# kasirershahartau/tissue_image_processing

Hardware: AMD Instinct MI355X
Metric: frames/sec end-to-end (2048^2, z=30) (higher is better)
Workload: dtype f32(f16x3)

## Files before the change

### tissue_image_processing_amd/csrc/tip_core.hip

```cpp
#include "tip_internal.h"
#include <algorithm>
#include <cmath>
#include <cstdlib>
#include <map>
#include <mutex>

namespace tip {

static thread_local Ctx *g_ctx = nullptr;
static thread_local int g_requested_device = 0;

static int ctx_create(int device)
{
    Ctx *c = new Ctx();
    c->device = device;
    hipError_t e = hipSetDevice(device);
    if (e != hipSuccess) {
        c->err = std::string("hipSetDevice failed: ") + hipGetErrorString(e);
        g_ctx = c;
        return TIP_ERR_HIP;
    }
    {
        const char *pr = getenv("TIP_STREAM_PRIORITY");
        int lo = 0, hi = 0;
// ... 107 lines not shown
namespace {
Tuning g_tuning;
std::once_flag g_tuning_once;
std::mutex g_tuning_mu;

bool tuning_assign(Tuning &t, const char *name, const char *value)
{
    const Tuning def;
    const bool unset = !value || !*value;
    auto flag = [&](int &field, int dflt) { field = unset ? dflt : (strcmp(value, "0") != 0 ? 1 : 0); };
    auto num = [&](int &field, int dflt) { field = unset ? dflt : atoi(value); };
    auto pair = [&](int &a, int &b, int da, int db) {
        a = da; b = db;
        if (!unset) sscanf(value, "%d,%d", &a, &b);
    };
    const std::string n(name ? name : "");
    if (n == "TIP_WS_TIES") {
        if (unset) t.ws_ties = def.ws_ties;
        else t.ws_ties = (!strcmp(value, "fast") || !strcmp(value, "0")) ? 0 : 1;
    }
    else if (n == "TIP_WS_OPEN") pair(t.ws_open_a, t.ws_open_b, def.ws_open_a, def.ws_open_b);
    else if (n == "TIP_WS_NO_SKIP") flag(t.ws_no_skip, 0);
    else if (n == "TIP_WS_DEBUG") flag(t.ws_debug, 0);
    else if (n == "TIP_WS_NO_ENDGAME") flag(t.ws_no_endgame, 0);
    else if (n == "TIP_WS_NO_WIDE") flag(t.ws_no_wide, 0);
    else if (n == "TIP_PROJECT_GENERIC") flag(t.project_generic, 0);
    else if (n == "TIP_PROJECT_UNFUSED_PREBLUR") flag(t.project_unfused_preblur, 0);
    else if (n == "TIP_PROJECT_UNFUSED_MASK") flag(t.project_unfused_mask, 0);
    else if (n == "TIP_PROJECT_EXACT_SCORE") flag(t.project_exact_score, 0);
    else if (n == "TIP_PROJECT_DEBUG") flag(t.project_debug, 0);
    else if (n == "TIP_UNET_TILE8") num(t.unet_tile8, def.unet_tile8);
    else if (n == "TIP_UF_ONE_LEVEL") flag(t.uf_one_level, 0);
    else if (n == "TIP_UNET_SPB") num(t.unet_spb, def.unet_spb);
    else if (n == "TIP_UNET_XCD_MAP") flag(t.unet_xcd_map, 1);
    else if (n == "TIP_UNET_TAIL_UNFUSED") flag(t.unet_tail_unfused, 0);
    else if (n == "TIP_MB_SMALL") num(t.mb_small, def.mb_small);
    else if (n == "TIP_MB_BATCH") num(t.mb_batch, def.mb_batch);
    else return false;
    return true;
}

const char *const TUNING_NAMES[] = {"TIP_WS_TIES", "TIP_WS_OPEN", "TIP_WS_NO_SKIP", "TIP_WS_DEBUG", "TIP_WS_NO_ENDGAME", "TIP_WS_NO_WIDE",
                                    "TIP_PROJECT_GENERIC", "TIP_PROJECT_UNFUSED_PREBLUR", "TIP_PROJECT_UNFUSED_MASK",
                                    "TIP_PROJECT_EXACT_SCORE", "TIP_PROJECT_DEBUG", "TIP_UNET_TILE8", "TIP_UNET_TAIL_UNFUSED", "TIP_UNET_XCD_MAP", "TIP_UNET_SPB", "TIP_UF_ONE_LEVEL", "TIP_MB_SMALL", "TIP_MB_BATCH"};

void tuning_from_env()
{
    for (const char *name : TUNING_NAMES)
        if (const char *e = getenv(name)) tuning_assign(g_tuning, name, e);
}
}

const Tuning &tuning()
{
    std::call_once(g_tuning_once, tuning_from_env);
    return g_tuning;
}

int make_taps(Taps &t, const double *w, int n)
{
    if (n <= 0 || n > 255 || !(n & 1)) return fail(TIP_ERR_ARG, "tap count %d must be odd and <= 255", n);
    for (int i = 1; i <= n / 2; i++)
        if (fabs(w[n / 2 + i] - w[n / 2 - i]) > 2.220446049250313e-16)
            return fail(TIP_ERR_UNSUPPORTED, "only symmetric kernels (scipy's symmetric correlate1d branch)");
    memset(&t, 0, sizeof t);
    for (int i = 0; i < n; i++) t.w[i] = w[i];
    t.n = n;
    return TIP_OK;
}

static double np_pairwise_sum(const double *a, long n)
{
    if (n < 8) {
        double r = 0.0;
        for (long i = 0; i < n; i++) r += a[i];
        return r;
    } else if (n <= 128) {
// ... 207 lines not shown
```

### tissue_image_processing_amd/csrc/tip_internal.h

```cpp
#pragma once
#include <hip/hip_runtime.h>
#include <cstdarg>
#include <cstdint>
#include <cstdio>
#include <cstring>
#include <string>
#include <vector>
#include "../../include/tissue_hip.h"

namespace tip {

struct ProfRec { const char *name; hipEvent_t e0, e1; };

struct Ctx {
    int device = -1;
    hipStream_t stream = nullptr;
    std::string err;
    struct Block { void *p; size_t bytes; bool used; };
    std::vector<Block> pool;
    int last_ws_labels = 0;
    long last_ws_other = 0;
    hipEvent_t edge_event = nullptr;
    void *prep_ws = nullptr;
    void *pin_buf = nullptr;
// ... 6 lines not shown
Ctx &ctx();
int fail(int code, const char *fmt, ...);
void *ws_alloc(size_t bytes);
void *pinned_scratch(size_t bytes);
void ws_free(void *p);

struct WsGuard {
    std::vector<void *> ptrs;
    template <typename T> T *get(size_t count) {
        void *p = ws_alloc(count * sizeof(T) ? count * sizeof(T) : 16);
        if (p) ptrs.push_back(p);
        return (T *)p;
    }
    ~WsGuard() { for (void *p : ptrs) ws_free(p); }
};

void prof_begin(const char *name);
void prof_end();

struct Tuning {
    int ws_ties = 1;
    int ws_open_a = -1, ws_open_b = -1;
    int ws_no_skip = 0;
    int ws_debug = 0;
    int ws_no_endgame = 0, ws_no_wide = 0;
    int project_generic = 0, project_unfused_preblur = 0, project_unfused_mask = 0;
    int project_exact_score = 0, project_debug = 0;
    int unet_tail_unfused = 0;
    int unet_xcd_map = 1;
    int unet_spb = 3;
    int uf_one_level = 0;
    int mb_small = -1;
    int mb_batch = -1;
    int unet_tile8 = -1;
};
const Tuning &tuning();

#define TIP_HIP(call)                                                                             \
    do {                                                                                          \
        hipError_t e__ = (call);                                                                  \
        if (e__ != hipSuccess)                                                                    \
            return tip::fail(TIP_ERR_HIP, "%s failed: %s (%s:%d)", #call, hipGetErrorString(e__), \
                             __FILE__, __LINE__);                                                 \
    } while (0)

#define TIP_LAUNCH(name, kernel, grid, block, shmem, ...)                                  \
    do {                                                                                   \
        tip::prof_begin(name);                                                             \
        hipLaunchKernelGGL(kernel, grid, block, shmem, tip::ctx().stream, __VA_ARGS__);    \
        tip::prof_end();                                                                   \
        hipError_t e__ = hipGetLastError();                                                \
        if (e__ != hipSuccess)                                                             \
            return tip::fail(TIP_ERR_HIP, "launch %s: %s", name, hipGetErrorString(e__));  \
    } while (0)

static inline int cdiv(long a, long b) { return (int)((a + b - 1) / b); }

struct Taps {
    double w[256];
    int n;
};
struct TapsF {
    float w[256];
    int n;
};

// ... 9 lines not shown
```

### tissue_image_processing_amd/csrc/tip_unet.hip

```cpp
#include "tip_internal.h"
#include "tip_unet_conv.h"
#include <algorithm>
#include <atomic>

namespace tip {

__global__ void __launch_bounds__(256) k_bias_relu_affine_f32(float *__restrict__ x, const float *__restrict__ bias,
                                                              const float *__restrict__ scale, const float *__restrict__ shift,
                                                              long n4, int C)
{
    const long i = (long)blockIdx.x * blockDim.x + threadIdx.x;
    if (i >= n4) return;
    float4 v = reinterpret_cast<float4 *>(x)[i];
    const int c = (int)((i * 4) % C);
    const float4 b = *reinterpret_cast<const float4 *>(bias + c);
    const float4 s = *reinterpret_cast<const float4 *>(scale + c);
    const float4 t = *reinterpret_cast<const float4 *>(shift + c);
    v.x += b.x; v.y += b.y; v.z += b.z; v.w += b.w;
    v.x = v.x > 0.f ? v.x : 0.f; v.y = v.y > 0.f ? v.y : 0.f; v.z = v.z > 0.f ? v.z : 0.f; v.w = v.w > 0.f ? v.w : 0.f;
    v.x = v.x * s.x + t.x; v.y = v.y * s.y + t.y; v.z = v.z * s.z + t.z; v.w = v.w * s.w + t.w;
    reinterpret_cast<float4 *>(x)[i] = v;
}

int rankfilter2d_dev(const void *in, void *out, int dtype, int Y, int X, int ky, int kx, int fp, int border, int is_max);
// ... 380 lines not shown
    p.in0 = (const uint16_t *)d->in0; p.in1 = (const uint16_t *)(d->c1 > 0 ? d->in1 : d->in0);
    p.c0 = d->c0; p.c1 = d->c1; p.H = d->h; p.W = d->w;
    p.w = (const uint16_t *)d->weights; p.ntaps = d->ntaps;
    for (int t = 0; t < 9; ++t) {
        p.dy[t] = t < d->ntaps ? d->dy[t] : 0; p.dx[t] = t < d->ntaps ? d->dx[t] : 0;
        if (p.dy[t] < -1 || p.dy[t] > 1 || p.dx[t] < -1 || p.dx[t] > 1) return fail(TIP_ERR_ARG, "tip_unet_conv_dev: tap offsets are -1, 0 or 1");
    }
    p.cout = d->cout; p.bias = d->bias; p.scale = d->scale; p.shift = d->shift;
    p.out = (uint16_t *)d->out; p.outH = d->out_h; p.outW = d->out_w; p.sy = d->sy; p.sx = d->sx; p.oy = d->oy; p.ox = d->ox;
    p.pool_out = (uint16_t *)d->pool_out;
    p.acc_scale = d->format == 1 ? d->acc_scale : 1.f;
    for (int t = 0; t < 9; ++t) p.nmask[t] = d->tf ? (d->nmask[t] & 15) : 15;
    if (d->tf && (d->planes != 2 || d->ntaps != 4 || d->sy != 2 || d->sx != 2 || d->oy != 0 || d->ox != 0 || d->scale || d->pool_out || d->head_out ||
                  d->out_h != 2 * d->h || d->out_w != 2 * d->w))
        return fail(TIP_ERR_ARG, "tip_unet_conv_dev: the fused transposed convolution takes four offset taps, two planes, bias only, a 2h x 2w output");
#ifdef UC_TRACE
    static unsigned long long *trace_dev = nullptr;
    if (!trace_dev) { TIP_HIP(hipMalloc(&trace_dev, 1024)); }
    TIP_HIP(hipMemsetAsync(trace_dev, 0, 1024, (hipStream_t)stream));
    p.trace = trace_dev;
#endif
    p.head_w = d->head_w; p.head_b = d->head_b; p.head_out = d->head_out;
    if (d->head_out && (!d->head_w || !d->head_b || d->cout != UC_BN || !d->scale || d->pool_out || d->sy != 1 || d->sx != 1 || d->oy != 0 || d->ox != 0 ||
                        d->out_h != d->h || d->out_w != d->w))
        return fail(TIP_ERR_ARG, "tip_unet_conv_dev: the fused head needs a 128-channel Conv2D + BatchNorm layer with the plain output mapping");
    if (d->pool_out && (d->sy != 1 || d->sx != 1 || d->oy != 0 || d->ox != 0 || d->out_h != d->h || d->out_w != d->w))
        return fail(TIP_ERR_ARG, "tip_unet_conv_dev: pool_out needs the plain output mapping");
    const bool tf = d->tf != 0;
    const int t8 = tuning().unet_tile8;
    const bool want8 = t8 == 1 || (t8 < 0 && d->ntaps == 9 && d->c0 + d->c1 <= 128);
    const int th = (d->planes == 2 && d->h % 16 == 0 && !want8) ? 16 : 8;
    const int dist = (th == 16 && d->ntaps >= 4) ? 4 : 2;
    const int da = (th == 16 && d->ntaps <= 2) ? 2 : 1;
    const int threads = th * 32, hp = UC_HW * (th + 2);
    const int ntiles = (d->h / th) * (d->w / UC_TW), nblks = d->cout / UC_BN;
    p.xcd_map = (tuning().unet_xcd_map && nblks > 1 && ntiles % 8 == 0) ? 1 : 0;
    const dim3 grid = p.xcd_map ? dim3((unsigned)(ntiles * nblks)) : dim3(ntiles, nblks);
    const int a_per = (d->planes * ((hp * 2 + 63) / 64) * 64 + threads - 1) / threads;
    const int spb_want = tuning().unet_spb;
    const bool multi = th == 16 && dist == 4 && d->ntaps == 9 && spb_want > 1;
    const int spb = !multi ? 1 : (spb_want >= 3 ? 3 : ((((d->c0 + d->c1) / UC_KC) & 1) == 0 ? 2 : 1));
    const size_t lds = (size_t)(da + 1) * a_per * threads * 16 + (size_t)(spb > 1 ? 3 * spb : dist + 1) * d->planes * 256 * 16;
    hipStream_t s = (hipStream_t)stream;
    const int which = tf ? (th == 16 ? 7 : 8)
                         : d->planes == 3 ? 3 : (th == 16 ? (dist == 4 ? (spb == 3 ? 6 : (spb == 2 ? 5 : 2)) : (da == 2 ? 4 : 1)) : 0);
    static std::atomic<unsigned> attr_done[64];
    const unsigned bit = 1u << (which + (d->format ? 9 : 0));
    const int dev = c.device >= 0 && c.device < 64 ? c.device : 0;
#define UC_FLAVOUR(W, ...)                                                                                                                  \
    case W: {                                                                                                                               \
        if (!(attr_done[dev].load(std::memory_order_acquire) & bit)) {                                                                      \
            TIP_HIP(hipFuncSetAttribute((const void *)(__VA_ARGS__), hipFuncAttributeMaxDynamicSharedMemorySize, (int)lds));                \
            attr_done[dev].fetch_or(bit, std::memory_order_release);                                                                        \
        }                                                                                                                                   \
        hipLaunchKernelGGL((__VA_ARGS__), grid, dim3(threads), lds, s, p);                                                                  \
    } break;
    if (d->format == 0) {
        switch (which) {
            UC_FLAVOUR(3, k_unet_conv<3, 8, 2>)
            UC_FLAVOUR(6, k_unet_conv<2, 16, 4, 1, 3>)
            UC_FLAVOUR(5, k_unet_conv<2, 16, 4, 1, 2>)
            UC_FLAVOUR(2, k_unet_conv<2, 16, 4>)
            UC_FLAVOUR(4, k_unet_conv<2, 16, 2, 2>)
            UC_FLAVOUR(1, k_unet_conv<2, 16, 2>)
            UC_FLAVOUR(0, k_unet_conv<2, 8, 2>)
            UC_FLAVOUR(7, k_unet_conv<2, 16, 4, 1, 1, false, true>)
            UC_FLAVOUR(8, k_unet_conv<2, 8, 2, 1, 1, false, true>)
        }
    } else {
        switch (which) {
            UC_FLAVOUR(6, k_unet_conv<2, 16, 4, 1, 3, true>)
            UC_FLAVOUR(5, k_unet_conv<2, 16, 4, 1, 2, true>)
            UC_FLAVOUR(2, k_unet_conv<2, 16, 4, 1, 1, true>)
            UC_FLAVOUR(4, k_unet_conv<2, 16, 2, 2, 1, true>)
            UC_FLAVOUR(1, k_unet_conv<2, 16, 2, 1, 1, true>)
            UC_FLAVOUR(0, k_unet_conv<2, 8, 2, 1, 1, true>)
            UC_FLAVOUR(7, k_unet_conv<2, 16, 4, 1, 1, true, true>)
            UC_FLAVOUR(8, k_unet_conv<2, 8, 2, 1, 1, true, true>)
        }
    }
#undef UC_FLAVOUR
#ifdef UC_TRACE
    {
        unsigned long long tr[128];
        TIP_HIP(hipStreamSynchronize(s));
        TIP_HIP(hipMemcpy(tr, trace_dev, sizeof tr, hipMemcpyDeviceToHost));
        for (int k = 0; k < th / 2; ++k) {
            const unsigned long long *t = tr + 16 * k;
            const double n = (double)t[4];
            fprintf(stderr, "UC_TRACE th %d spb %d taps %d cin %d cout %d grid %dx%d wave %d simd %d: per STEP (shader clocks; sums over the loop / steps): copies %.0f, products %.0f (first MFMA out after %.0f), "
                            "vmcnt wait %.0f, barrier %.0f, total %.0f; steps %.0f; whole loop %.0f, prologue %.0f, epilogue %.0f clocks\n",
                    th, spb, d->ntaps, d->c0 + d->c1, d->cout, d->h, d->w, k, (int)((t[7] >> 4) & 3), t[0] / n, t[2] / n, t[1] / n, t[6] / n, (t[3] - t[6]) / n, t[5] / n, n, (double)t[5], (double)t[8], (double)t[9]);
        }
    }
#endif
    return unet_launch_check("unet_conv");
}

int tip_unet_conv_first_dev(const float *in, int h, int w, const float *wgt, const float *bias, const float *scale, const float *shift,
                            void *out, int planes, int format, void *stream)
{
    Ctx &c = ctx();
    if (!c.stream) return TIP_ERR_HIP;
    if (!in || !wgt || !bias || !scale || !shift || !out || h < 1 || w < 1 || w % FIRST_RUN || ((long)h * w) % FIRST_PIX || (planes != 2 && planes != 3) ||
        (format != 0 && !(format == 1 && planes == 2)))
        return fail(TIP_ERR_ARG, "tip_unet_conv_first_dev: bad arguments (w must be a multiple of 32, h * w of 256)");
    const dim3 grid((unsigned)((long)h * w / FIRST_PIX));
    hipStream_t s = (hipStream_t)stream;
    if (format == 1) hipLaunchKernelGGL((k_unet_conv_first<2, true>), grid, dim3(256), 0, s, in, h, w, wgt, bias, scale, shift, (uint16_t *)out);
    else if (planes == 2) hipLaunchKernelGGL(k_unet_conv_first<2>, grid, dim3(256), 0, s, in, h, w, wgt, bias, scale, shift, (uint16_t *)out);
    else hipLaunchKernelGGL(k_unet_conv_first<3>, grid, dim3(256), 0, s, in, h, w, wgt, bias, scale, shift, (uint16_t *)out);
// ... 33 lines not shown
```

### tissue_image_processing_amd/csrc/tip_unet_conv.h

```cpp
#pragma once
#include "tip_internal.h"

namespace tip {

typedef __bf16 bf16x8 __attribute__((ext_vector_type(8)));
typedef float f32x16 __attribute__((ext_vector_type(16)));
typedef __bf16 bf16x2 __attribute__((ext_vector_type(2)));
typedef float f32x2 __attribute__((ext_vector_type(2)));
typedef _Float16 f16x8 __attribute__((ext_vector_type(8)));
typedef _Float16 f16x2 __attribute__((ext_vector_type(2)));
constexpr float UC_F16_MAX = 65504.f;

constexpr int UC_TW = 32;
constexpr int UC_BN = 128;
constexpr int UC_KC = 16;
constexpr int UC_HW = UC_TW + 2;

struct ConvParams {
    const uint16_t *in0, *in1;
    int c0, c1;
    int H, W;
    const uint16_t *w;
    int ntaps;
    int dy[9], dx[9];
// ... 10 lines not shown
    float acc_scale;
    int nmask[9];
    uint16_t *pool_out;
};

__device__ __forceinline__ unsigned bf16_rne_bits(float v)
{
    const unsigned b = __float_as_uint(v);
    return (b + 0x7fffu + ((b >> 16) & 1u)) >> 16;
}
__device__ __forceinline__ float bf16_bits_to_f32(unsigned h) { return __uint_as_float(h << 16); }
__device__ __forceinline__ float relu_bits(float v) { return __int_as_float(max(__float_as_int(v), 0)); }
__device__ __forceinline__ float fmax_raw(float a, float b)
{
    float r;
    asm("v_max_f32 %0, %1, %2" : "=v"(r) : "v"(a), "v"(b));
    return r;
}
__device__ __forceinline__ float fmax_pair(float v)
{
    float r;
    asm("s_nop 1\n\tv_max_f32_dpp %0, %1, %1 quad_perm:[1,0,3,2] row_mask:0xf bank_mask:0xf" : "=v"(r) : "v"(v));
    return r;
}

typedef __attribute__((address_space(3))) unsigned char lds_byte;

template <bool F16>
__device__ __forceinline__ f32x16 uc_mfma(const uint4 &a, const uint4 &b, const f32x16 &c)
{
    if constexpr (F16) return __builtin_amdgcn_mfma_f32_32x32x16_f16(__builtin_bit_cast(f16x8, a), __builtin_bit_cast(f16x8, b), c, 0, 0, 0);
    else return __builtin_amdgcn_mfma_f32_32x32x16_bf16(__builtin_bit_cast(bf16x8, a), __builtin_bit_cast(bf16x8, b), c, 0, 0, 0);
}
template <bool F16>
__device__ __forceinline__ unsigned uc_piece_word(float &a, float &b, bool more)
{
    if constexpr (F16) {
        f16x2 hv;
        hv[0] = (_Float16)a;
        hv[1] = (_Float16)b;
        if (more) {
            a -= (float)hv[0];
            b -= (float)hv[1];
        }
        return __builtin_bit_cast(unsigned, hv);
    } else {
        bf16x2 hv;
        hv[0] = (__bf16)a;
        hv[1] = (__bf16)b;
        const unsigned w = __builtin_bit_cast(unsigned, hv);
        if (more) {
            const f32x2 r = f32x2{a, b} - f32x2{__uint_as_float(w << 16), __uint_as_float(w & 0xffff0000u)};
            a = r[0];
            b = r[1];
        }
        return w;
    }
}
template <bool F16>
__device__ __forceinline__ float uc_piece_value(unsigned halfword)
{
    if constexpr (F16) return (float)__builtin_bit_cast(_Float16, (unsigned short)halfword);
    else return __uint_as_float(halfword << 16);
}
__device__ __forceinline__ float uc_sat_f16(float v) { return __builtin_amdgcn_fmed3f(v, -UC_F16_MAX, UC_F16_MAX); }

#ifdef UC_TRACE
__device__ unsigned long long uc_trace_wait_ticks;
template <int N>
__device__ __forceinline__ unsigned long long uc_wait_barrier_timed()
{
    asm volatile("s_waitcnt vmcnt(%0) lgkmcnt(0)" ::"n"(N) : "memory");
    const unsigned long long t = __builtin_amdgcn_s_memtime();
    asm volatile("s_waitcnt lgkmcnt(0)\n\ts_barrier" ::: "memory");
    return t;
}
#endif
template <int N>
__device__ __forceinline__ void uc_wait_barrier()
{
    asm volatile("s_waitcnt vmcnt(%0) lgkmcnt(0)\n\ts_barrier" ::"n"(N) : "memory");
}

template <int NPL, int TH, int D, int DA = 1, int SPB = 1, bool F16 = false, bool TF = false>
__global__ void __launch_bounds__(TH * 32, (NPL == 2) ? 2 : 1) k_unet_conv(const ConvParams p)
{
#if defined(__HIP_DEVICE_COMPILE__)
#ifdef UC_TRACE
    const unsigned long long tr_enter = __builtin_amdgcn_s_memtime();
#endif
    static_assert(DA == 1 || (DA == 2 && D == 2), "two-chunk activation prefetch: with the two-step weight schedule");
    static_assert(SPB == 1 || ((SPB == 2 || SPB == 3) && D == 4 && DA == 1 && TH == 16), "several steps per barrier: the 16-row kernel with the four-step weight schedule");
    constexpr bool PAIR = SPB > 1;
    constexpr int UC_NBBUF = PAIR ? 3 * SPB : D + 1;
    constexpr int UC_THREADS = TH * 32, UC_HP = UC_HW * (TH + 2);
    static_assert(TH == 8 || (TH == 16 && NPL == 2), "16-row tiles: two pieces (LDS)");
    static_assert(!TF || (NPL == 2 && SPB == 1), "fused transposed convolution: two pieces, one step per barrier");
    constexpr int A_GPP = (UC_HP * 2 + 63) / 64, A_PLANE = A_GPP * 64;
    constexpr int A_PER = (NPL * A_PLANE + UC_THREADS - 1) / UC_THREADS;
    constexpr int A_SLOTS = A_PER * UC_THREADS;
    constexpr int A_BYTES = A_SLOTS * 16;
    constexpr int B_PER = NPL * 256 / UC_THREADS;
    static_assert(B_PER * UC_THREADS == NPL * 256, "weight slots divide evenly");
    constexpr int B_BYTES = NPL * 256 * 16;
    extern __shared__ __attribute__((aligned(16))) unsigned char smem[];
    unsigned char *sA = smem, *sB = smem + (DA + 1) * A_BYTES;
    const int tid = threadIdx.x, lane = tid & 63;
    const int wave = __builtin_amdgcn_readfirstlane(tid >> 6);
    const int tilesX = p.W / UC_TW;
    const int nblks = p.cout / UC_BN;
    int tile, nblk;
    if (p.xcd_map) {
        const int b = blockIdx.x, xcd = b & 7, j = b >> 3;
        tile = (j / nblks) * 8 + xcd;
        nblk = j - (j / nblks) * nblks;
    } else {
        tile = blockIdx.x;
        nblk = blockIdx.y;
    }
    const int ty0 = (tile / tilesX) * TH, tx0 = (tile % tilesX) * UC_TW;
    const int cin = p.c0 + p.c1, nchunks = cin / UC_KC, nsteps = nchunks * p.ntaps;
    const long in_plane0 = (long)p.H * p.W * p.c0, in_plane1 = (long)p.H * p.W * p.c1;
    const int rowbase = ty0 > 0 ? ty0 - 1 : 0;
    const int winrows = min(p.H, ty0 + TH + 1) - rowbase;

    unsigned a_off[A_PER];
    auto plan_a = [&](int C) {
#pragma unroll
        for (int u = 0; u < A_PER; ++u) {
            const int g = u * (UC_THREADS / 64) + wave, pl = g / A_GPP;
            const int rem = (g - pl * A_GPP) * 64 + lane, px = rem >> 1, half = (rem & 1) ^ ((px >> 3) & 1);
            const int hy = px / UC_HW, hx = px - hy * UC_HW;
            const int gy = ty0 + hy - 1, gx = tx0 + hx - 1;
            const bool inside = pl < NPL && rem < UC_HP * 2 && gy >= 0 && gy < p.H && gx >= 0 && gx < p.W;
            a_off[u] = inside ? (unsigned)((((long)(gy - rowbase) * p.W + gx) * C + half * 8) * 2) : 0xffff0000u;
        }
    };
    plan_a(p.c0);
    bool a_second = false;
    constexpr int RSRC_FLAGS = 0x00020000;
    unsigned long long a_win = (unsigned long long)(p.in0 + (long)rowbase * p.W * p.c0), a_plane_bytes = (unsigned long long)in_plane0 * 2;
    int a_rec = (int)(unsigned)((long)winrows * p.W * p.c0 * 2);
    const __amdgpu_buffer_rsrc_t rs_b = __builtin_amdgcn_make_buffer_rsrc((void *)p.w, 0, (int)0xffffffffu, RSRC_FLAGS);
    auto copy_a = [&](int chunk, int buf) {
        const int cbase = chunk * UC_KC;
        const bool second = cbase >= p.c0;
        if (second && !a_second) {
            a_second = true;
            a_win = (unsigned long long)(p.in1 + (long)rowbase * p.W * p.c1);
            a_plane_bytes = (unsigned long long)in_plane1 * 2;
            a_rec = (int)(unsigned)((long)winrows * p.W * p.c1 * 2);
            if (p.c1 != p.c0) plan_a(p.c1);
        }
        const int soff = (second ? cbase - p.c0 : cbase) * 2;
        lds_byte *dst = (lds_byte *)(sA + buf * A_BYTES + wave * 64 * 16);
#pragma unroll
        for (int u = 0; u < A_PER; ++u) {
            const int pl = min((u * (UC_THREADS / 64) + wave) / A_GPP, NPL - 1);
            const unsigned long long base = a_win + (unsigned long long)pl * a_plane_bytes;
            const unsigned lo = __builtin_amdgcn_readfirstlane((unsigned)base), hi = __builtin_amdgcn_readfirstlane((unsigned)(base >> 32));
            const __amdgpu_buffer_rsrc_t rs = __builtin_amdgcn_make_buffer_rsrc((void *)(((unsigned long long)hi << 32) | lo), 0, __builtin_amdgcn_readfirstlane(a_rec), RSRC_FLAGS);
            __builtin_amdgcn_raw_ptr_buffer_load_lds(rs, dst + u * UC_THREADS * 16, 16, a_off[u], soff, 0, 0);
        }
    };
    const int bq = tid & 255;
    const unsigned b_off = (unsigned)(((tid >> 8) * (UC_BN * UC_KC) + (bq >> 1) * UC_KC + (((bq & 1) ^ ((bq >> 4) & 1))) * 8) * 2);
    auto copy_b = [&](int chunk, int tap, int buf) {
        const int soff = ((tap * nchunks + chunk) * nblks + nblk) * (NPL * UC_BN * UC_KC * 2);
        lds_byte *dst = (lds_byte *)(sB + buf * B_BYTES + wave * 64 * 16);
#pragma unroll
        for (int u = 0; u < B_PER; ++u)
            __builtin_amdgcn_raw_ptr_buffer_load_lds(rs_b, dst + u * UC_THREADS * 16, 16, b_off, soff + u * (UC_THREADS / 256) * (UC_BN * UC_KC * 2), 0, 0);
    };

    f32x16 acc[2][4];
#pragma unroll
    for (int m = 0; m < 2; ++m)
#pragma unroll
        for (int n = 0; n < 4; ++n)
#pragma unroll
            for (int i = 0; i < 16; ++i) acc[m][n][i] = 0.f;

    copy_a(0, 0);
    if (DA == 2 && nchunks > 1) copy_a(1, 1);
    for (int s0 = 0; s0 < (PAIR ? 2 * SPB : D) && s0 < nsteps; ++s0) copy_b(s0 / p.ntaps, s0 % p.ntaps, s0);
    uc_wait_barrier<0>();

    const int r = lane & 31, h = lane >> 5;
    const int b_row = r * 2 + (h ^ ((r >> 3) & 1));
    int step = 0;
    int nc = D / p.ntaps, nt = D % p.ntaps;
    int buf0 = 0, buf2 = D;
    uint4 fa[2][NPL], fb[4][NPL];
#ifdef UC_TRACE
    unsigned long long tr_copy = 0, tr_read = 0, tr_mfma = 0, tr_bar = 0, tr_t0 = __builtin_amdgcn_s_memtime();
    const bool tracing = blockIdx.x == gridDim.x / 2 && blockIdx.y == 0;
    unsigned long long tr_wait = 0, t_w = 0;
#define UC_T(var) const unsigned long long var = __builtin_amdgcn_s_memtime()
#define UC_WB t_w = uc_wait_barrier_timed
#else
#define UC_T(var)
#define UC_WB uc_wait_barrier
#endif
#define UC_PRODUCT(PA, PB)                                                                                      \
    _Pragma("unroll") for (int m = 0; m < 2; ++m) _Pragma("unroll") for (int n = 0; n < 4; ++n)                 \
        acc[m][n] = uc_mfma<F16>(fb[n][PB], fa[m][PA], acc[m][n]);
    auto step_products = [&](int chunk, int tap) {
        const unsigned char *abuf = sA + (chunk % (DA + 1)) * A_BYTES;
        const unsigned char *bbuf = sB + buf0 * B_BYTES;
        const int dy = p.dy[tap], dx = p.dx[tap];
// ... 29 lines not shown
            __builtin_amdgcn_s_setprio(1);
            acc[0][0] = uc_mfma<F16>(fb[0][0], fa[0][1], acc[0][0]);
            __builtin_amdgcn_sched_barrier(0);
            read_a(0, 0); read_a(1, 0);
#pragma unroll
            for (int n = 0; n < 4; ++n) read_b(n, 1);
            __builtin_amdgcn_sched_barrier(0);
#pragma unroll
            for (int n = 1; n < 4; ++n) acc[0][n] = uc_mfma<F16>(fb[n][0], fa[0][1], acc[0][n]);
#pragma unroll
            for (int n = 0; n < 4; ++n) acc[1][n] = uc_mfma<F16>(fb[n][0], fa[1][1], acc[1][n]);
            __builtin_amdgcn_sched_barrier(0);
#ifndef UC_TWO_PRODUCTS
            UC_PRODUCT(0, 1)
#endif
            UC_PRODUCT(0, 0)
            __builtin_amdgcn_s_setprio(0);
        } else {
#pragma unroll
            for (int k = 0; k < NPL; ++k) {
#pragma unroll
                for (int m = 0; m < 2; ++m) read_a(m, NPL - 1 - k);
#pragma unroll
                for (int n = 0; n < 4; ++n) read_b(n, k);
            }
            __builtin_amdgcn_s_setprio(1);
            UC_PRODUCT(2, 0) UC_PRODUCT(1, 1) UC_PRODUCT(0, 2)
            UC_PRODUCT(1, 0)
            UC_PRODUCT(0, 1)
            UC_PRODUCT(0, 0)
            __builtin_amdgcn_s_setprio(0);
        }
    };
    if constexpr (PAIR) {
        int c0 = 0, t0 = 0;
        int cb = (2 * SPB) / p.ntaps, tb = (2 * SPB) % p.ntaps;
        int bb = 0;
        int a_issued = 0;
        auto next = [&](int &c, int &t) { if (++t == p.ntaps) { t = 0; ++c; } };
        auto wrapb = [](int b) { return b >= UC_NBBUF ? b - UC_NBBUF : b; };
        for (int s = 0; s < nsteps; s += SPB) {
            UC_T(t_a);
            const bool issue_a = c0 + 1 < nchunks && c0 + 1 > a_issued;
            const int ca = c0 + 1;
            if (issue_a) a_issued = ca;
            const bool issue_b = s + 2 * SPB < nsteps;
            UC_T(t_b);
#pragma unroll
            for (int k = 0; k < SPB; ++k) {
                buf0 = wrapb(bb + k);
                step_products(c0, t0);
                next(c0, t0);
                if (k == 0 && issue_a) copy_a(ca, ca & 1);
                if (issue_b) { copy_b(cb, tb, wrapb(bb + 2 * SPB + k)); next(cb, tb); }
            }
            UC_T(t_c);
            if (issue_b) { if (issue_a) UC_WB<A_PER + SPB * B_PER>(); else UC_WB<SPB * B_PER>(); }
            else { if (issue_a) UC_WB<A_PER>(); else UC_WB<0>(); }
            bb = wrapb(bb + SPB);
#ifdef UC_TRACE
            UC_T(t_d);
            tr_copy += t_b - t_a; tr_mfma += t_c - t_b; tr_bar += t_d - t_c; tr_wait += t_w - t_c;
#endif
        }
    } else
    for (int chunk = 0; chunk < nchunks; ++chunk) {
        for (int tap = 0; tap < p.ntaps; ++tap, ++step) {
// ... 37 lines not shown
    if (tracing && p.trace && lane == 0) {
        unsigned long long *tp = p.trace + 16 * wave;
        tp[0] = tr_copy; tp[1] = tr_read; tp[2] = tr_mfma; tp[3] = tr_bar; tp[4] = (unsigned long long)nsteps;
        tp[5] = __builtin_amdgcn_s_memtime() - tr_t0; tp[6] = tr_wait; tp[7] = (unsigned long long)__builtin_amdgcn_s_getreg((31 << 11) | 4);
        tp[8] = tr_t0 - tr_enter;
    }
    const unsigned long long tr_loop_end = __builtin_amdgcn_s_memtime();
#endif
#undef UC_PRODUCT

    constexpr int EP_ROW = 272, EP_BYTES = 32 * EP_ROW;
    static_assert(UC_THREADS / 64 * EP_BYTES <= (DA + 1) * A_BYTES + UC_NBBUF * B_BYTES, "the staging images fit the tile buffers");
    int pxl = lane & 31, hf = lane >> 5;
    asm volatile("" : "+v"(pxl), "+v"(hf));
    unsigned char *ep = smem + wave * EP_BYTES;
    {
        const float *bip = p.bias + nblk * UC_BN + 16 * hf;
        const float *scp = p.scale + nblk * UC_BN + 16 * hf, *shp = p.shift + nblk * UC_BN + 16 * hf;
        const f32x2 inv2 = {p.acc_scale, p.acc_scale};
        auto biased = [&](float a0, float a1, const f32x2 &b) -> f32x2 {
            if constexpr (F16) return __builtin_elementwise_fma(f32x2{a0, a1}, inv2, b);
            else return f32x2{a0, a1} + b;
        };
#pragma unroll
        for (int n = 0; n < 4; ++n) {
#pragma unroll
            for (int q = 0; q < 4; ++q) {
                const float4 b4 = *reinterpret_cast<const float4 *>(bip + n * 32 + q * 4);
                const f32x2 b01 = {b4.x, b4.y}, b23 = {b4.z, b4.w};
                if (p.scale) {
                    const float4 s4 = *reinterpret_cast<const float4 *>(scp + n * 32 + q * 4), t4 = *reinterpret_cast<const float4 *>(shp + n * 32 + q * 4);
                    const f32x2 s01 = {s4.x, s4.y}, s23 = {s4.z, s4.w}, t01 = {t4.x, t4.y}, t23 = {t4.z, t4.w};
#pragma unroll
                    for (int m = 0; m < 2; ++m) {
                        f32x2 v01 = biased(acc[m][n][q * 4 + 0], acc[m][n][q * 4 + 1], b01);
                        f32x2 v23 = biased(acc[m][n][q * 4 + 2], acc[m][n][q * 4 + 3], b23);
                        v01 = __builtin_elementwise_fma(f32x2{relu_bits(v01[0]), relu_bits(v01[1])}, s01, t01);
                        v23 = __builtin_elementwise_fma(f32x2{relu_bits(v23[0]), relu_bits(v23[1])}, s23, t23);
                        if constexpr (F16) {
                            v01 = f32x2{uc_sat_f16(v01[0]), uc_sat_f16(v01[1])};
                            v23 = f32x2{uc_sat_f16(v23[0]), uc_sat_f16(v23[1])};
                        }
                        acc[m][n][q * 4 + 0] = v01[0]; acc[m][n][q * 4 + 1] = v01[1];
                        acc[m][n][q * 4 + 2] = v23[0]; acc[m][n][q * 4 + 3] = v23[1];
                    }
                } else {
#pragma unroll
                    for (int m = 0; m < 2; ++m) {
                        f32x2 v01 = biased(acc[m][n][q * 4 + 0], acc[m][n][q * 4 + 1], b01);
                        f32x2 v23 = biased(acc[m][n][q * 4 + 2], acc[m][n][q * 4 + 3], b23);
                        if constexpr (F16) {
                            v01 = f32x2{uc_sat_f16(v01[0]), uc_sat_f16(v01[1])};
                            v23 = f32x2{uc_sat_f16(v23[0]), uc_sat_f16(v23[1])};
                        }
                        acc[m][n][q * 4 + 0] = v01[0]; acc[m][n][q * 4 + 1] = v01[1];
                        acc[m][n][q * 4 + 2] = v23[0]; acc[m][n][q * 4 + 3] = v23[1];
                    }
                }
            }
            asm volatile("" ::: "memory");
        }
    }
    if (p.head_out) {
        float z[2][2] = {{0.f, 0.f}, {0.f, 0.f}};
        const float *hw0 = p.head_w + 16 * hf, *hw1 = p.head_w + UC_BN + 16 * hf;
#pragma unroll
        for (int n = 0; n < 4; ++n)
#pragma unroll
            for (int q = 0; q < 4; ++q) {
                const float4 a4 = *reinterpret_cast<const float4 *>(hw0 + n * 32 + q * 4), b4 = *reinterpret_cast<const float4 *>(hw1 + n * 32 + q * 4);
                const float wa[4] = {a4.x, a4.y, a4.z, a4.w}, wb[4] = {b4.x, b4.y, b4.z, b4.w};
#pragma unroll
                for (int m = 0; m < 2; ++m)
#pragma unroll
                    for (int j = 0; j < 4; ++j) {
                        z[m][0] = __builtin_fmaf(acc[m][n][q * 4 + j], wa[j], z[m][0]);
                        z[m][1] = __builtin_fmaf(acc[m][n][q * 4 + j], wb[j], z[m][1]);
                    }
            }
#pragma unroll
        for (int m = 0; m < 2; ++m)
#pragma unroll
            for (int c = 0; c < 2; ++c) z[m][c] += __shfl_xor(z[m][c], 32, 64);
        const float z0 = (hf ? z[1][0] : z[0][0]) + p.head_b[0], z1 = (hf ? z[1][1] : z[0][1]) + p.head_b[1];
        const float zm = z0 > z1 ? z0 : z1;
        const float e0 = __expf(z0 - zm), e1 = __expf(z1 - zm);
        const float es = e0 + e1;
        const long o = (long)(ty0 + wave * 2 + hf) * p.W + tx0 + pxl;
        p.head_out[o] = e0 / es;
        p.head_out[(long)p.H * p.W + o] = e1 / es;
        return;
    }
    auto piece_word = [](float &a, float &b, bool more) -> unsigned { return uc_piece_word<F16>(a, b, more); };
    const int rd_row = lane >> 4, rd_col = (lane & 15) * 16;
    const long out_plane = (long)p.outH * p.outW * (TF ? p.cout / 4 : p.cout);
    if (p.pool_out) {
        const long pool_plane = (long)(p.outH / 2) * (p.outW / 2) * p.cout;
        const bool oddp = pxl & 1;
        float q8[4][8];
#pragma unroll
        for (int n = 0; n < 4; ++n)
#pragma unroll
            for (int i = 0; i < 16; ++i) {
                const float v = fmax_pair(fmax_raw(acc[0][n][i], acc[1][n][i]));
                if (i < 8) q8[n][i] = v; else if (oddp) q8[n][i - 8] = v;
            }
        uint16_t *prow = p.pool_out + ((long)(ty0 / 2 + wave) * (p.outW / 2) + tx0 / 2) * p.cout + nblk * UC_BN + (lane & 15) * 8;
#pragma unroll
        for (int pl = 0; pl < NPL; ++pl) {
#pragma unroll
            for (int n = 0; n < 4; ++n) {
                uint4 w;
                w.x = piece_word(q8[n][0], q8[n][1], pl + 1 < NPL);
                w.y = piece_word(q8[n][2], q8[n][3], pl + 1 < NPL);
                w.z = piece_word(q8[n][4], q8[n][5], pl + 1 < NPL);
                w.w = piece_word(q8[n][6], q8[n][7], pl + 1 < NPL);
                *reinterpret_cast<uint4 *>(ep + (pxl >> 1) * EP_ROW + (n * 32 + 16 * hf + (oddp ? 8 : 0)) * 2) = w;
            }
#pragma unroll
            for (int it = 0; it < 4; ++it) {
                const int row = it * 4 + rd_row;
                *reinterpret_cast<uint4 *>(prow + pl * pool_plane + (long)row * p.cout) = *reinterpret_cast<const uint4 *>(ep + row * EP_ROW + rd_col);
            }
        }
    }
#pragma unroll
    for (int m = 0; m < 2; ++m) {
        const int y = ty0 + wave * 2 + m;
        const int cls = (lane & 15) >> 2;
        const long pix_stride = TF ? p.cout / 4 : p.cout;
        uint16_t *orow = TF ? p.out + ((long)(2 * y + (cls >> 1)) * p.outW + (2 * (long)tx0 + (cls & 1))) * pix_stride + nblk * 32 + (lane & 3) * 8
                            : p.out + ((long)(y * p.sy + p.oy) * p.outW + ((long)tx0 * p.sx + p.ox)) * p.cout + nblk * UC_BN + (lane & 15) * 8;
#pragma unroll
        for (int pl = 0; pl < NPL; ++pl) {
#pragma unroll
            for (int n = 0; n < 4; ++n)
#pragma unroll
                for (int q = 0; q < 2; ++q) {
                    float v[8];
#pragma unroll
                    for (int j = 0; j < 8; ++j) v[j] = acc[m][n][q * 8 + j];
                    uint4 w;
                    w.x = piece_word(v[0], v[1], pl + 1 < NPL);
                    w.y = piece_word(v[2], v[3], pl + 1 < NPL);
                    w.z = piece_word(v[4], v[5], pl + 1 < NPL);
                    w.w = piece_word(v[6], v[7], pl + 1 < NPL);
                    if (pl + 1 < NPL) {
#pragma unroll
                        for (int j = 0; j < 8; ++j) acc[m][n][q * 8 + j] = v[j];
                    }
                    *reinterpret_cast<uint4 *>(ep + pxl * EP_ROW + (n * 32 + 16 * hf + 8 * q) * 2) = w;
                }
#pragma unroll
            for (int it = 0; it < 8; ++it) {
                const int row = it * 4 + rd_row;
                *reinterpret_cast<uint4 *>(orow + pl * out_plane + (long)row * p.sx * pix_stride) = *reinterpret_cast<const uint4 *>(ep + row * EP_ROW + rd_col);
            }
        }
    }
#ifdef UC_TRACE
    if (tracing && p.trace && lane == 0) {
// ... 170 lines not shown
```

Measured before the change: 18.84.

## Add four-wave UNet 3x3 conv variant with four rows per wave and AGPR MFMA accumulation

Adds a W4 flavour of the UNet convolution kernel that uses 256 threads for 16-row tiles, so each wave computes four output rows instead of two. Its main loop is hand-scheduled: MFMAs accumulate directly into AGPRs via inline asm, and LDS fragment reads and async global-to-LDS copies are interleaved between individual MFMAs. The aim is to reuse each B fragment across more rows and keep the matrix units busy with fewer waves. In exchange it roughly doubles accumulator registers per wave and drops to one block per CU. It also depends on fragile manual scheduling and trailing s_nop hazard padding. It is enabled by default for wide-channel layers (c0+c1 >= 256) with 9 taps.

Result: no change. 18.66, median of 3 (-1.0%).

```diff
diff --git a/tissue_image_processing_amd/csrc/tip_core.hip b/tissue_image_processing_amd/csrc/tip_core.hip
--- a/tissue_image_processing_amd/csrc/tip_core.hip
+++ b/tissue_image_processing_amd/csrc/tip_core.hip
@@ -163,6 +163,7 @@
     else if (n == "TIP_UNET_TILE8") num(t.unet_tile8, def.unet_tile8);
     else if (n == "TIP_UF_ONE_LEVEL") flag(t.uf_one_level, 0);
     else if (n == "TIP_UNET_SPB") num(t.unet_spb, def.unet_spb);
+    else if (n == "TIP_UNET_WAVE4") num(t.unet_wave4, def.unet_wave4);
     else if (n == "TIP_UNET_XCD_MAP") flag(t.unet_xcd_map, 1);
     else if (n == "TIP_UNET_TAIL_UNFUSED") flag(t.unet_tail_unfused, 0);
     else if (n == "TIP_MB_SMALL") num(t.mb_small, def.mb_small);
@@ -173,7 +174,7 @@
 
 const char *const TUNING_NAMES[] = {"TIP_WS_TIES", "TIP_WS_OPEN", "TIP_WS_NO_SKIP", "TIP_WS_DEBUG", "TIP_WS_NO_ENDGAME", "TIP_WS_NO_WIDE",
                                     "TIP_PROJECT_GENERIC", "TIP_PROJECT_UNFUSED_PREBLUR", "TIP_PROJECT_UNFUSED_MASK",
-                                    "TIP_PROJECT_EXACT_SCORE", "TIP_PROJECT_DEBUG", "TIP_UNET_TILE8", "TIP_UNET_TAIL_UNFUSED", "TIP_UNET_XCD_MAP", "TIP_UNET_SPB", "TIP_UF_ONE_LEVEL", "TIP_MB_SMALL", "TIP_MB_BATCH"};
+                                    "TIP_PROJECT_EXACT_SCORE", "TIP_PROJECT_DEBUG", "TIP_UNET_TILE8", "TIP_UNET_TAIL_UNFUSED", "TIP_UNET_XCD_MAP", "TIP_UNET_SPB", "TIP_UNET_WAVE4", "TIP_UF_ONE_LEVEL", "TIP_MB_SMALL", "TIP_MB_BATCH"};
 
 void tuning_from_env()
 {
diff --git a/tissue_image_processing_amd/csrc/tip_internal.h b/tissue_image_processing_amd/csrc/tip_internal.h
--- a/tissue_image_processing_amd/csrc/tip_internal.h
+++ b/tissue_image_processing_amd/csrc/tip_internal.h
@@ -62,6 +62,7 @@
     int uf_one_level = 0;
     int mb_small = -1;
     int mb_batch = -1;
+    int unet_wave4 = -1;
     int unet_tile8 = -1;
 };
 const Tuning &tuning();
diff --git a/tissue_image_processing_amd/csrc/tip_unet.hip b/tissue_image_processing_amd/csrc/tip_unet.hip
--- a/tissue_image_processing_amd/csrc/tip_unet.hip
+++ b/tissue_image_processing_amd/csrc/tip_unet.hip
@@ -436,7 +436,10 @@
     const int th = (d->planes == 2 && d->h % 16 == 0 && !want8) ? 16 : 8;
     const int dist = (th == 16 && d->ntaps >= 4) ? 4 : 2;
     const int da = (th == 16 && d->ntaps <= 2) ? 2 : 1;
-    const int threads = th * 32, hp = UC_HW * (th + 2);
+    const int w4_want = tuning().unet_wave4;
+    const bool w4 = !tf && th == 16 && dist == 4 && d->ntaps == 9 && tuning().unet_spb >= 3 &&
+                    (w4_want == 1 || (w4_want < 0 && d->c0 + d->c1 >= 256));
+    const int threads = w4 ? 256 : th * 32, hp = UC_HW * (th + 2);
     const int ntiles = (d->h / th) * (d->w / UC_TW), nblks = d->cout / UC_BN;
     p.xcd_map = (tuning().unet_xcd_map && nblks > 1 && ntiles % 8 == 0) ? 1 : 0;
     const dim3 grid = p.xcd_map ? dim3((unsigned)(ntiles * nblks)) : dim3(ntiles, nblks);
@@ -446,10 +449,10 @@
     const int spb = !multi ? 1 : (spb_want >= 3 ? 3 : ((((d->c0 + d->c1) / UC_KC) & 1) == 0 ? 2 : 1));
     const size_t lds = (size_t)(da + 1) * a_per * threads * 16 + (size_t)(spb > 1 ? 3 * spb : dist + 1) * d->planes * 256 * 16;
     hipStream_t s = (hipStream_t)stream;
-    const int which = tf ? (th == 16 ? 7 : 8)
+    const int which = w4 ? 9 : tf ? (th == 16 ? 7 : 8)
                          : d->planes == 3 ? 3 : (th == 16 ? (dist == 4 ? (spb == 3 ? 6 : (spb == 2 ? 5 : 2)) : (da == 2 ? 4 : 1)) : 0);
     static std::atomic<unsigned> attr_done[64];
-    const unsigned bit = 1u << (which + (d->format ? 9 : 0));
+    const unsigned bit = 1u << (which + (d->format ? 10 : 0));
     const int dev = c.device >= 0 && c.device < 64 ? c.device : 0;
 #define UC_FLAVOUR(W, ...)                                                                                                                  \
     case W: {                                                                                                                               \
@@ -470,6 +473,7 @@
             UC_FLAVOUR(0, k_unet_conv<2, 8, 2>)
             UC_FLAVOUR(7, k_unet_conv<2, 16, 4, 1, 1, false, true>)
             UC_FLAVOUR(8, k_unet_conv<2, 8, 2, 1, 1, false, true>)
+            UC_FLAVOUR(9, k_unet_conv<2, 16, 4, 1, 3, false, false, true>)
         }
     } else {
         switch (which) {
@@ -481,6 +485,7 @@
             UC_FLAVOUR(0, k_unet_conv<2, 8, 2, 1, 1, true>)
             UC_FLAVOUR(7, k_unet_conv<2, 16, 4, 1, 1, true, true>)
             UC_FLAVOUR(8, k_unet_conv<2, 8, 2, 1, 1, true, true>)
+            UC_FLAVOUR(9, k_unet_conv<2, 16, 4, 1, 3, true, false, true>)
         }
     }
 #undef UC_FLAVOUR
diff --git a/tissue_image_processing_amd/csrc/tip_unet_conv.h b/tissue_image_processing_amd/csrc/tip_unet_conv.h
--- a/tissue_image_processing_amd/csrc/tip_unet_conv.h
+++ b/tissue_image_processing_amd/csrc/tip_unet_conv.h
@@ -66,6 +66,14 @@
     if constexpr (F16) return __builtin_amdgcn_mfma_f32_32x32x16_f16(__builtin_bit_cast(f16x8, a), __builtin_bit_cast(f16x8, b), c, 0, 0, 0);
     else return __builtin_amdgcn_mfma_f32_32x32x16_bf16(__builtin_bit_cast(bf16x8, a), __builtin_bit_cast(bf16x8, b), c, 0, 0, 0);
 }
+typedef unsigned u32x4 __attribute__((ext_vector_type(4)));
+template <bool F16>
+__device__ __forceinline__ void uc_mfma_agpr(const uint4 &a, const uint4 &b, f32x16 &c)
+{
+    if constexpr (F16) asm volatile("v_mfma_f32_32x32x16_f16 %0, %1, %2, %0" : "+a"(c) : "v"(__builtin_bit_cast(u32x4, a)), "v"(__builtin_bit_cast(u32x4, b)));
+    else asm volatile("v_mfma_f32_32x32x16_bf16 %0, %1, %2, %0" : "+a"(c) : "v"(__builtin_bit_cast(u32x4, a)), "v"(__builtin_bit_cast(u32x4, b)));
+}
+__device__ __forceinline__ void uc_mfma_settle() { asm volatile("s_nop 15\n\ts_nop 15" ::: "memory"); }
 template <bool F16>
 __device__ __forceinline__ unsigned uc_piece_word(float &a, float &b, bool more)
 {
@@ -116,8 +124,8 @@
     asm volatile("s_waitcnt vmcnt(%0) lgkmcnt(0)\n\ts_barrier" ::"n"(N) : "memory");
 }
 
-template <int NPL, int TH, int D, int DA = 1, int SPB = 1, bool F16 = false, bool TF = false>
-__global__ void __launch_bounds__(TH * 32, (NPL == 2) ? 2 : 1) k_unet_conv(const ConvParams p)
+template <int NPL, int TH, int D, int DA = 1, int SPB = 1, bool F16 = false, bool TF = false, bool W4 = false>
+__global__ void __launch_bounds__(W4 ? 256 : TH * 32, (NPL == 2 && !W4) ? 2 : 1) k_unet_conv(const ConvParams p)
 {
 #if defined(__HIP_DEVICE_COMPILE__)
 #ifdef UC_TRACE
@@ -127,7 +135,9 @@
     static_assert(SPB == 1 || ((SPB == 2 || SPB == 3) && D == 4 && DA == 1 && TH == 16), "several steps per barrier: the 16-row kernel with the four-step weight schedule");
     constexpr bool PAIR = SPB > 1;
     constexpr int UC_NBBUF = PAIR ? 3 * SPB : D + 1;
-    constexpr int UC_THREADS = TH * 32, UC_HP = UC_HW * (TH + 2);
+    constexpr int UC_THREADS = W4 ? 256 : TH * 32, UC_HP = UC_HW * (TH + 2);
+    constexpr int RPW = W4 ? 4 : 2;
+    static_assert(!W4 || (TH == 16 && NPL == 2 && SPB == 3 && !TF), "four-wave tile: the 3x3 kernel with three steps per barrier");
     static_assert(TH == 8 || (TH == 16 && NPL == 2), "16-row tiles: two pieces (LDS)");
     static_assert(!TF || (NPL == 2 && SPB == 1), "fused transposed convolution: two pieces, one step per barrier");
     constexpr int A_GPP = (UC_HP * 2 + 63) / 64, A_PLANE = A_GPP * 64;
@@ -176,7 +186,7 @@
     unsigned long long a_win = (unsigned long long)(p.in0 + (long)rowbase * p.W * p.c0), a_plane_bytes = (unsigned long long)in_plane0 * 2;
     int a_rec = (int)(unsigned)((long)winrows * p.W * p.c0 * 2);
     const __amdgpu_buffer_rsrc_t rs_b = __builtin_amdgcn_make_buffer_rsrc((void *)p.w, 0, (int)0xffffffffu, RSRC_FLAGS);
-    auto copy_a = [&](int chunk, int buf) {
+    auto copy_a_open = [&](int chunk) -> int {
         const int cbase = chunk * UC_KC;
         const bool second = cbase >= p.c0;
         if (second && !a_second) {
@@ -186,30 +196,36 @@
             a_rec = (int)(unsigned)((long)winrows * p.W * p.c1 * 2);
             if (p.c1 != p.c0) plan_a(p.c1);
         }
-        const int soff = (second ? cbase - p.c0 : cbase) * 2;
+        return (second ? cbase - p.c0 : cbase) * 2;
+    };
+    auto copy_a_one = [&](int u, int soff, int buf) {
         lds_byte *dst = (lds_byte *)(sA + buf * A_BYTES + wave * 64 * 16);
-#pragma unroll
-        for (int u = 0; u < A_PER; ++u) {
-            const int pl = min((u * (UC_THREADS / 64) + wave) / A_GPP, NPL - 1);
-            const unsigned long long base = a_win + (unsigned long long)pl * a_plane_bytes;
-            const unsigned lo = __builtin_amdgcn_readfirstlane((unsigned)base), hi = __builtin_amdgcn_readfirstlane((unsigned)(base >> 32));
-            const __amdgpu_buffer_rsrc_t rs = __builtin_amdgcn_make_buffer_rsrc((void *)(((unsigned long long)hi << 32) | lo), 0, __builtin_amdgcn_readfirstlane(a_rec), RSRC_FLAGS);
-            __builtin_amdgcn_raw_ptr_buffer_load_lds(rs, dst + u * UC_THREADS * 16, 16, a_off[u], soff, 0, 0);
-        }
+        const int pl = min((u * (UC_THREADS / 64) + wave) / A_GPP, NPL - 1);
+        const unsigned long long base = a_win + (unsigned long long)pl * a_plane_bytes;
+        const unsigned lo = __builtin_amdgcn_readfirstlane((unsigned)base), hi = __builtin_amdgcn_readfirstlane((unsigned)(base >> 32));
+        const __amdgpu_buffer_rsrc_t rs = __builtin_amdgcn_make_buffer_rsrc((void *)(((unsigned long long)hi << 32) | lo), 0, __builtin_amdgcn_readfirstlane(a_rec), RSRC_FLAGS);
+        __builtin_amdgcn_raw_ptr_buffer_load_lds(rs, dst + u * UC_THREADS * 16, 16, a_off[u], soff, 0, 0);
+    };
+    auto copy_a = [&](int chunk, int buf) {
+        const int soff = copy_a_open(chunk);
+#pragma unroll
+        for (int u = 0; u < A_PER; ++u) copy_a_one(u, soff, buf);
     };
     const int bq = tid & 255;
     const unsigned b_off = (unsigned)(((tid >> 8) * (UC_BN * UC_KC) + (bq >> 1) * UC_KC + (((bq & 1) ^ ((bq >> 4) & 1))) * 8) * 2);
-    auto copy_b = [&](int chunk, int tap, int buf) {
+    auto copy_b_one = [&](int u, int chunk, int tap, int buf) {
         const int soff = ((tap * nchunks + chunk) * nblks + nblk) * (NPL * UC_BN * UC_KC * 2);
         lds_byte *dst = (lds_byte *)(sB + buf * B_BYTES + wave * 64 * 16);
-#pragma unroll
-        for (int u = 0; u < B_PER; ++u)
-            __builtin_amdgcn_raw_ptr_buffer_load_lds(rs_b, dst + u * UC_THREADS * 16, 16, b_off, soff + u * (UC_THREADS / 256) * (UC_BN * UC_KC * 2), 0, 0);
+        __builtin_amdgcn_raw_ptr_buffer_load_lds(rs_b, dst + u * UC_THREADS * 16, 16, b_off, soff + u * (UC_THREADS / 256) * (UC_BN * UC_KC * 2), 0, 0);
     };
-
-    f32x16 acc[2][4];
-#pragma unroll
-    for (int m = 0; m < 2; ++m)
+    auto copy_b = [&](int chunk, int tap, int buf) {
+#pragma unroll
+        for (int u = 0; u < B_PER; ++u) copy_b_one(u, chunk, tap, buf);
+    };
+
+    f32x16 acc[RPW][4];
+#pragma unroll
+    for (int m = 0; m < RPW; ++m)
 #pragma unroll
         for (int n = 0; n < 4; ++n)
 #pragma unroll
@@ -305,7 +321,85 @@
             __builtin_amdgcn_s_setprio(0);
         }
     };
-    if constexpr (PAIR) {
+    if constexpr (W4) {
+        unsigned long long tapcode = 0;
+        for (int t = 0; t < p.ntaps; ++t) tapcode |= (unsigned long long)((p.dy[t] + 1) | ((p.dx[t] + 1) << 2)) << (4 * t);
+        uint4 fa4[2][4][2], fb4[2][4][2];
+        int c0 = 0, t0 = 0;
+        int cb = (2 * SPB) / p.ntaps, tb = (2 * SPB) % p.ntaps;
+        int bb = 0;
+        int a_issued = 0;
+        auto next = [&](int &c, int &t) { if (++t == p.ntaps) { t = 0; ++c; } };
+        auto wrapb = [](int b) { return b >= UC_NBBUF ? b - UC_NBBUF : b; };
+        auto frag_offsets = [&](int chunk, int tap, int wb, unsigned (&ao)[4], unsigned &bo) {
+            const int code = (int)(tapcode >> (4 * tap)) & 15, dy = (code & 3) - 1, dx = (code >> 2) - 1;
+            const int px0 = (wave * 4 + 1 + dy) * UC_HW + (r + 1 + dx);
+#pragma unroll
+            for (int m = 0; m < 4; ++m) {
+                const int px = px0 + m * UC_HW;
+                ao[m] = (unsigned)((chunk & 1) * A_BYTES + (px * 2 + (h ^ ((px >> 3) & 1))) * 16);
+            }
+            bo = (unsigned)((DA + 1) * A_BYTES + wb * B_BYTES + b_row * 16);
+        };
+        auto read_frag = [&](int S, int i, const unsigned (&ao)[4], unsigned bo) {
+            auto ra = [&](int m, int pl) { fa4[S][m][pl] = *reinterpret_cast<const uint4 *>(smem + ao[m] + pl * (A_PLANE * 16)); };
+            auto rb = [&](int n, int pl) { fb4[S][n][pl] = *reinterpret_cast<const uint4 *>(smem + bo + (pl * 256 + n * 64) * 16); };
+            if (i == 0) ra(0, 1);
+            else if (i < 5) rb(i - 1, 0);
+            else if (i < 8) ra(i - 4, 1);
+            else if (i < 12) ra(i - 8, 0);
+            else rb(i - 12, 1);
+        };
+        auto iteration = [&](const bool IA, const bool IB, int ca, int a_soff) {
+            unsigned ao[4], bo, an[4], bn;
+            frag_offsets(c0, t0, bb, ao, bo);
+#pragma unroll
+            for (int i = 0; i < 8; ++i) read_frag(0, i, ao, bo);
+            __builtin_amdgcn_sched_barrier(0);
+#pragma unroll
+            for (int k = 0; k < SPB; ++k) {
+                const int S = k & 1;
+                next(c0, t0);
+                if (k + 1 < SPB) frag_offsets(c0, t0, wrapb(bb + k + 1), an, bn);
+                __builtin_amdgcn_sched_barrier(0);
+#pragma unroll
+                for (int j = 0; j < 16; ++j) {
+                    uc_mfma_agpr<F16>(fb4[S][j & 3][0], fa4[S][j >> 2][1], acc[j >> 2][j & 3]);
+                    if (k == 0) { if (j < 8) read_frag(0, 8 + j, ao, bo); else read_frag(1, j - 8, an, bn); }
+                    else if (k + 1 < SPB) read_frag(S ^ 1, j, an, bn);
+                    __builtin_amdgcn_sched_barrier(0);
+                }
+#pragma unroll
+                for (int j = 0; j < 16; ++j) {
+                    uc_mfma_agpr<F16>(fb4[S][j & 3][1], fa4[S][j >> 2][0], acc[j >> 2][j & 3]);
+                    const int ja = (k == 0 && IA) ? A_PER : 0;
+                    static_assert(A_PER + B_PER <= 16, "a step's copies pair up with one product group");
+                    if (j < ja) copy_a_one(j, a_soff, ca & 1);
+                    else if (IB && j < ja + B_PER) copy_b_one(j - ja, cb, tb, wrapb(bb + 2 * SPB + k));
+                    __builtin_amdgcn_sched_barrier(0);
+                }
+                if (IB) next(cb, tb);
+#pragma unroll
+                for (int j = 0; j < 16; ++j) {
+                    uc_mfma_agpr<F16>(fb4[S][j & 3][0], fa4[S][j >> 2][0], acc[j >> 2][j & 3]);
+                    if (k == 0 && j < 8) { read_frag(1, 8 + j, an, bn); __builtin_amdgcn_sched_barrier(0); }
+                }
+                __builtin_amdgcn_sched_barrier(0);
+            }
+            if (IB) { if (IA) uc_wait_barrier<A_PER + SPB * B_PER>(); else uc_wait_barrier<SPB * B_PER>(); }
+            else { if (IA) uc_wait_barrier<A_PER>(); else uc_wait_barrier<0>(); }
+            bb = wrapb(bb + SPB);
+        };
+        for (int s = 0; s < nsteps; s += SPB) {
+            const bool issue_a = c0 + 1 < nchunks && c0 + 1 > a_issued;
+            const int ca = c0 + 1;
+            int a_soff = 0;
+            if (issue_a) { a_issued = ca; a_soff = copy_a_open(ca); }
+            const bool issue_b = s + 2 * SPB < nsteps;
+            iteration(issue_a, issue_b, ca, a_soff);
+        }
+        uc_mfma_settle();
+    } else if constexpr (PAIR) {
         int c0 = 0, t0 = 0;
         int cb = (2 * SPB) / p.ntaps, tb = (2 * SPB) % p.ntaps;
         int bb = 0;
@@ -409,7 +503,7 @@
                     const float4 s4 = *reinterpret_cast<const float4 *>(scp + n * 32 + q * 4), t4 = *reinterpret_cast<const float4 *>(shp + n * 32 + q * 4);
                     const f32x2 s01 = {s4.x, s4.y}, s23 = {s4.z, s4.w}, t01 = {t4.x, t4.y}, t23 = {t4.z, t4.w};
 #pragma unroll
-                    for (int m = 0; m < 2; ++m) {
+                    for (int m = 0; m < RPW; ++m) {
                         f32x2 v01 = biased(acc[m][n][q * 4 + 0], acc[m][n][q * 4 + 1], b01);
                         f32x2 v23 = biased(acc[m][n][q * 4 + 2], acc[m][n][q * 4 + 3], b23);
                         v01 = __builtin_elementwise_fma(f32x2{relu_bits(v01[0]), relu_bits(v01[1])}, s01, t01);
@@ -423,7 +517,7 @@
                     }
                 } else {
 #pragma unroll
-                    for (int m = 0; m < 2; ++m) {
+                    for (int m = 0; m < RPW; ++m) {
                         f32x2 v01 = biased(acc[m][n][q * 4 + 0], acc[m][n][q * 4 + 1], b01);
                         f32x2 v23 = biased(acc[m][n][q * 4 + 2], acc[m][n][q * 4 + 3], b23);
                         if constexpr (F16) {
@@ -439,7 +533,9 @@
         }
     }
     if (p.head_out) {
-        float z[2][2] = {{0.f, 0.f}, {0.f, 0.f}};
+        float z[RPW][2];
+#pragma unroll
+        for (int m = 0; m < RPW; ++m) z[m][0] = z[m][1] = 0.f;
         const float *hw0 = p.head_w + 16 * hf, *hw1 = p.head_w + UC_BN + 16 * hf;
 #pragma unroll
         for (int n = 0; n < 4; ++n)
@@ -448,7 +544,7 @@
                 const float4 a4 = *reinterpret_cast<const float4 *>(hw0 + n * 32 + q * 4), b4 = *reinterpret_cast<const float4 *>(hw1 + n * 32 + q * 4);
                 const float wa[4] = {a4.x, a4.y, a4.z, a4.w}, wb[4] = {b4.x, b4.y, b4.z, b4.w};
 #pragma unroll
-                for (int m = 0; m < 2; ++m)
+                for (int m = 0; m < RPW; ++m)
 #pragma unroll
                     for (int j = 0; j < 4; ++j) {
                         z[m][0] = __builtin_fmaf(acc[m][n][q * 4 + j], wa[j], z[m][0]);
@@ -456,16 +552,19 @@
                     }
             }
 #pragma unroll
-        for (int m = 0; m < 2; ++m)
+        for (int m = 0; m < RPW; ++m)
 #pragma unroll
             for (int c = 0; c < 2; ++c) z[m][c] += __shfl_xor(z[m][c], 32, 64);
-        const float z0 = (hf ? z[1][0] : z[0][0]) + p.head_b[0], z1 = (hf ? z[1][1] : z[0][1]) + p.head_b[1];
-        const float zm = z0 > z1 ? z0 : z1;
-        const float e0 = __expf(z0 - zm), e1 = __expf(z1 - zm);
-        const float es = e0 + e1;
-        const long o = (long)(ty0 + wave * 2 + hf) * p.W + tx0 + pxl;
-        p.head_out[o] = e0 / es;
-        p.head_out[(long)p.H * p.W + o] = e1 / es;
+#pragma unroll
+        for (int mp = 0; mp < RPW; mp += 2) {
+            const float z0 = (hf ? z[mp + 1][0] : z[mp][0]) + p.head_b[0], z1 = (hf ? z[mp + 1][1] : z[mp][1]) + p.head_b[1];
+            const float zm = z0 > z1 ? z0 : z1;
+            const float e0 = __expf(z0 - zm), e1 = __expf(z1 - zm);
+            const float es = e0 + e1;
+            const long o = (long)(ty0 + wave * RPW + mp + hf) * p.W + tx0 + pxl;
+            p.head_out[o] = e0 / es;
+            p.head_out[(long)p.H * p.W + o] = e1 / es;
+        }
         return;
     }
     auto piece_word = [](float &a, float &b, bool more) -> unsigned { return uc_piece_word<F16>(a, b, more); };
@@ -474,15 +573,17 @@
     if (p.pool_out) {
         const long pool_plane = (long)(p.outH / 2) * (p.outW / 2) * p.cout;
         const bool oddp = pxl & 1;
+#pragma unroll
+        for (int mp = 0; mp < RPW / 2; ++mp) {
         float q8[4][8];
 #pragma unroll
         for (int n = 0; n < 4; ++n)
 #pragma unroll
             for (int i = 0; i < 16; ++i) {
-                const float v = fmax_pair(fmax_raw(acc[0][n][i], acc[1][n][i]));
+                const float v = fmax_pair(fmax_raw(acc[2 * mp][n][i], acc[2 * mp + 1][n][i]));
                 if (i < 8) q8[n][i] = v; else if (oddp) q8[n][i - 8] = v;
             }
-        uint16_t *prow = p.pool_out + ((long)(ty0 / 2 + wave) * (p.outW / 2) + tx0 / 2) * p.cout + nblk * UC_BN + (lane & 15) * 8;
+        uint16_t *prow = p.pool_out + ((long)(ty0 / 2 + wave * (RPW / 2) + mp) * (p.outW / 2) + tx0 / 2) * p.cout + nblk * UC_BN + (lane & 15) * 8;
 #pragma unroll
         for (int pl = 0; pl < NPL; ++pl) {
 #pragma unroll
@@ -500,10 +601,11 @@
                 *reinterpret_cast<uint4 *>(prow + pl * pool_plane + (long)row * p.cout) = *reinterpret_cast<const uint4 *>(ep + row * EP_ROW + rd_col);
             }
         }
-    }
-#pragma unroll
-    for (int m = 0; m < 2; ++m) {
-        const int y = ty0 + wave * 2 + m;
+        }
+    }
+#pragma unroll
+    for (int m = 0; m < RPW; ++m) {
+        const int y = ty0 + wave * RPW + m;
         const int cls = (lane & 15) >> 2;
         const long pix_stride = TF ? p.cout / 4 : p.cout;
         uint16_t *orow = TF ? p.out + ((long)(2 * y + (cls >> 1)) * p.outW + (2 * (long)tx0 + (cls & 1))) * pix_stride + nblk * 32 + (lane & 3) * 8
```
